# CederGroupHub/sparse-lm

Measured on AMD Instinct MI355X. Metric: fits/sec over 50-alpha Lasso path at n=100k p=5k, higher is better.
Workload: dtype f64

## Files before the change

sparse-lm_amd/csrc/engine_path.hip:

```cpp
#include "engine_internal.hpp"

static int ws_policy(const slm_host::Knobs& kn, const slm_dataset* ds, uint32_t flags) {
  if (ds->max_group > WS_KCAP / 2 || ds->n < 4) return 0;
  if (kn.ws == 0 || (flags & SLM_FLAG_NO_WORKING_SET)) return 0;
  const bool big = (double)ds->n * (double)ds->ld >= 67108864.0;
  return (big || (flags & SLM_FLAG_WORKING_SET) || kn.ws == 1) ? 2 : 1;
}

static bool small_ok(const slm_host::Knobs& kn, const slm_dataset* ds, uint32_t flags) {
  if (!(flags & SLM_FLAG_ON_CHIP)) return false;
  if (flags & (SLM_FLAG_NO_RESTART | SLM_FLAG_PROFILE | SLM_FLAG_FISTA_ONLY | SLM_FLAG_WORKING_SET | SLM_FLAG_NO_WORKING_SET))
    return false;
  if (!kn.on_chip) return false;
  return ds->p <= SM_PMAX && (double)ds->n * (double)ds->ld <= 131072.0 && !row_sharded(ds);
}
static bool split_possible(const slm_dataset* ds) {
  return ds->sk != nullptr && (ds->sk->rowdot != nullptr || !ds->XT_failed);
}
static int max_lanes_for(const slm_host::Knobs& kn, const slm_dataset* ds, uint32_t flags) {
  if (small_ok(kn, ds, flags)) return ds->lane_cap;
  if ((ws_policy(kn, ds, flags) == 2 || (double)ds->n * (double)ds->ld >= 67108864.0) && split_possible(ds)) {
    if (ws_policy(kn, ds, flags) == 2 && !row_sharded(ds) && ds->sk->rowdot != nullptr && !ds->XT_failed)
      return kMaxLanes;
    return SPLIT_LANES;
// ... 559 lines not shown
  ta.zprev = ds->zprev;
  ta.gprev = ds->gprev;
  ta.gscale = ds->gscale;
  ta.uscratch = ds->u;
  ta.a0 = ds->a0;
  ta.b0 = ds->b0;
  ta.d0 = ds->d0;
  ta.order = ds->order;
  ta.gid = ds->gid;
  ta.gstart = ds->gstart;
  ta.betas_out = ds->betas_out;
  ta.gn_out = any_gn ? ds->gn_out : nullptr;
  ta.infos = d_infos;

  return SLM_OK;
}

int PathCall::enqueue_result_copies() {
  int64_t at = 0;
  for (int l = 0; l < B;) {
    int l1 = l + 1;
    int64_t pts = lanes[l].n_points;
    const bool gn = lanes[l].group_norms_out != nullptr, inf = lanes[l].infos != nullptr;
    while (l1 < B && lanes[l1].betas_out == lanes[l].betas_out + (size_t)pts * p &&
           (lanes[l1].group_norms_out != nullptr) == gn && (lanes[l1].infos != nullptr) == inf &&
           (!gn || lanes[l1].group_norms_out == lanes[l].group_norms_out + (size_t)pts * G) &&
           (!inf || lanes[l1].infos == lanes[l].infos + pts)) {
      pts += lanes[l1].n_points;
      ++l1;
    }
    HIP_TRY(hipMemcpyAsync(lanes[l].betas_out, ds->betas_out + (size_t)at * p, sizeof(double) * (size_t)pts * p,
                           hipMemcpyDeviceToHost, s));
    if (gn)
      HIP_TRY(hipMemcpyAsync(lanes[l].group_norms_out, ds->gn_out + (size_t)at * G, sizeof(double) * (size_t)pts * G,
                             hipMemcpyDeviceToHost, s));
    if (inf && !infos_in_snap)
      HIP_TRY(hipMemcpyAsync(lanes[l].infos, ds->infos + at, sizeof(slm_point_info) * (size_t)pts,
                             hipMemcpyDeviceToHost, s));
    at += pts;
    l = l1;
  }
  return SLM_OK;
}

int PathCall::run_on_chip() {
  SmallArgs sm;
  memset(&sm, 0, sizeof(sm));
  sm.t = ta;
  sm.X = ds->X; sm.y = ds->y; sm.rw = ls.rw; sm.rw_stride = ls.rw_stride; sm.n = n;
  for (int l = 0; l < kMaxCells; ++l) sm.inv_n[l] = 1.0 / (ls.n_eff[l] > 0 ? ls.n_eff[l] : (double)ds->n_global);
  sm.max_iters = (int)std::min<int64_t>((int64_t)o.max_iter, 1500);
  sm.cold = (o.flags & SLM_FLAG_COLD_START) ? 1 : 0;
  const size_t fixed = sizeof(double) * ((size_t)p * p + 3 * (size_t)p);
  const size_t lds = (size_t)SM_LDS_BYTES;
  sm.stage_doubles = (int)((lds - fixed - 64) / sizeof(double));
  SLM_TRY(allow_big_lds((const void*)small_solve_kernel, eng->device));
  bool staged_out = (size_t)total_points * (size_t)p <= kSmallOutDoubles && !any_gn;
  if (staged_out && !ds->h_small_out &&
      hipHostMalloc((void**)&ds->h_small_out, sizeof(double) * kSmallOutDoubles, hipHostMallocDefault) != hipSuccess) {
    (void)hipGetLastError();
    ds->h_small_out = nullptr;
    staged_out = false;
  }
  if (staged_out) sm.t.betas_out = ds->h_small_out;
  hipLaunchKernelGGL(small_solve_kernel, dim3(B), dim3(SM_THREADS), lds, s, sm);
  SLM_TRY(check_launch());
  if (infos_in_snap) HIP_TRY(hipMemcpyAsync(&ds->hctl[0].c, ds->dctl, sizeof(DevCtl), hipMemcpyDeviceToHost, s));
  else HIP_TRY(hipMemcpyAsync(&ds->hctl[0].c, ds->dctl, offsetof(DevCtl, infos), hipMemcpyDeviceToHost, s));
  if (!staged_out) SLM_TRY(enqueue_result_copies());
  else if (!infos_in_snap) {
    int64_t at_i = 0;
    for (int l = 0; l < B; ++l) {
      if (lanes[l].infos)
        HIP_TRY(hipMemcpyAsync(lanes[l].infos, ds->infos + at_i, sizeof(slm_point_info) * (size_t)lanes[l].n_points, hipMemcpyDeviceToHost, s));
      at_i += lanes[l].n_points;
    }
  }
  HIP_TRY(hipStreamSynchronize(s));
  if (staged_out) {
    int64_t at_o = 0;
    for (int l = 0; l < B; ++l) {
      memcpy(lanes[l].betas_out, ds->h_small_out + (size_t)at_o * p, sizeof(double) * (size_t)lanes[l].n_points * p);
      at_o += lanes[l].n_points;
    }
  }
  const double t_small = t_mark();
  const DevCtl& snap = ds->hctl[0].c;
  bool nonfinite = false, unconverged = false;
  int64_t at = 0, sweeps = 0;
  std::vector<slm_point_info> far_infos;
  if (!infos_in_snap) {
    far_infos.resize((size_t)total_points);
    HIP_TRY(hipMemcpy(far_infos.data(), ds->infos, sizeof(slm_point_info) * (size_t)total_points, hipMemcpyDeviceToHost));
  }
  const slm_point_info* all = infos_in_snap ? snap.infos : far_infos.data();
  for (int l = 0; l < B; ++l) {
    nonfinite = nonfinite || snap.lane[l].nonfinite;
    sweeps += snap.lane[l].iter;
    for (int k = 0; k < lanes[l].n_points; ++k) unconverged = unconverged || all[at + k].status == SLM_ERR_NOT_CONVERGED;
    if (infos_in_snap && lanes[l].infos) memcpy(lanes[l].infos, snap.infos + at, sizeof(slm_point_info) * (size_t)lanes[l].n_points);
    at += lanes[l].n_points;
  }
  if (nonfinite) return fail(SLM_ERR_NON_FINITE, "non-finite iterate (diverged or non-finite data)");
  if (rules) {
    if (unconverged) return fail(SLM_ERR_UNSUPPORTED, "a re-weighted round was not settled on chip");
    for (int l = 0; l < B; ++l) {
      if (snap.lane[l].rounds < 1) return fail(SLM_ERR_UNSUPPORTED, "lane %d: the re-weighting rule covers no weight", l);
      rounds_out[l] = snap.lane[l].rounds;
    }
  }
  if (unconverged) {
    if (kn.trace == 2) fprintf(stderr, "[slm] on-chip solve gave a point up after %.3f ms (%lld products): the general path takes the call\n", t_small, (long long)sweeps);
    return solve_without_chip(kn, ds, lanes, B, o, stats, shared_path);
  }
  if (stats) {
    memset(stats, 0, sizeof(*stats));
    stats->grad_launches = 1;
    stats->ws_inner_iters = sweeps;
    stats->wall_ms = t_mark();
  }
  if (kn.trace == 2) {
      int sl = 0;
      double worst = -1.0;
      for (int l = 0; l < B; ++l) {
        const double t = snap.lane[l].hist[0] + snap.lane[l].hist[1] + snap.lane[l].hist[2] + snap.lane[l].hist[3] + snap.lane[l].hist[4];
        if (t > worst) { worst = t; sl = l; }
      }
      fprintf(stderr, "[slm] on-chip solve: row weights %.3f setup %.3f launched+synced %.3f end %.3f ms, %lld products; slowest lane (%d of %d, %d points, "
              "%d products, %d face solves) in the kernel: Gram %.3f, lambda_max %.3f, proximal steps %.3f, faces %.3f, records %.3f ms\n", tr_rw, tr[0],
              t_small, t_mark(), (long long)sweeps, sl, B, lanes[sl].n_points, snap.lane[sl].iter, (int)snap.lane[sl].n_hist, snap.lane[sl].hist[0],
              snap.lane[sl].hist[1], snap.lane[sl].hist[2], snap.lane[sl].hist[3], snap.lane[sl].hist[4]);
    }
  return SLM_OK;
}

int PathCall::ws_setup(bool late) {
  const int* set_of = ws_set_of;
  const int* set_lane = ws_set_lane;
  const int n_sets = ws_n_sets;
  const int ws_nblk_most = (int)std::max<int64_t>(1, std::min<int64_t>(eng->cus, n / 64));
  const bool share_blocks = ls.rw != nullptr && !sharded && n_sets > 1;
  const int ws_nblk = share_blocks ? std::max(1, std::min(ws_nblk_most, eng->cus - 2 * n_sets)) : ws_nblk_most;
  if (!ds->ws_idx) SLM_TRY(dalloc(&ds->ws_idx, WS_KCAP));
  if (!ds->ws_gs) SLM_TRY(dalloc(&ds->ws_gs, WS_KCAP));
  if (!ds->ws_gl) SLM_TRY(dalloc(&ds->ws_gl, WS_KCAP));
  if (!ds->ws_pos) SLM_TRY(dalloc(&ds->ws_pos, (size_t)ld));
  if (!ds->ws_score) SLM_TRY(dalloc(&ds->ws_score, (size_t)ld));
  if (!ds->ws_XW) SLM_TRY(dalloc(&ds->ws_XW, (size_t)n * WS_KCAP));
  if (!ds->ws_nt) SLM_TRY(dalloc(&ds->ws_nt, (size_t)kMaxLanes * NT_SCRATCH));
  if (ds->ws_sets < n_sets) {
    dfree(ds->ws_part); dfree(ds->ws_G); dfree(ds->ws_Gx);
    ds->ws_sets = 0;
    if (sharded) SLM_TRY(dalloc(&ds->ws_Gx, (size_t)n_sets * WS_KCAP * WS_KCAP + STOP_WORDS));
    SLM_TRY(dalloc(&ds->ws_part, (size_t)ws_nblk_most * n_sets * WS_KCAP * WS_KCAP));
    SLM_TRY(dalloc(&ds->ws_G, (size_t)n_sets * WS_KCAP * WS_KCAP));
    ds->ws_sets = n_sets;
  }
  SLM_TRY(ensure_xt(kn, ds));
  if (late) HIP_TRY(hipMemsetAsync(ds->ws_ctl, 0, sizeof(WsCtl), s));
  if (ws_carry && !late) hipLaunchKernelGGL(ws_ctl_carry_kernel, dim3(1), dim3(256), 0, s, ds->ws_ctl, kWsMaxBuilds);
  else if (late || !ws_begun) hipLaunchKernelGGL(ws_ctl_init_kernel, dim3(1), dim3(64), 0, s, ds->ws_ctl, kWsMaxBuilds);
  wa.ws = ds->ws_ctl;
  wa.idx = ds->ws_idx; wa.pos = ds->ws_pos; wa.gs = ds->ws_gs; wa.gl = ds->ws_gl;
  wa.score = ds->ws_score; wa.XW = ds->ws_XW; wa.part = ds->ws_part; wa.Gm = ds->ws_G;
  wa.nt = ds->ws_nt;
  if (sharded && !ds->ws_Gx) SLM_TRY(dalloc(&ds->ws_Gx, (size_t)ds->ws_sets * WS_KCAP * WS_KCAP + STOP_WORDS));
  wa.Gx = sharded ? ds->ws_Gx : nullptr;
  wa.X = ds->X; wa.XT = ds->XT; wa.n = n; wa.ld = ld;
  wa.rw = ls.rw; wa.rw_stride = ls.rw_stride;
  for (int l = 0; l < kMaxLanes; ++l) {
    wa.set_of[l] = l < B ? set_of[l] : 0;
    wa.set_lane[l] = l < n_sets ? set_lane[l] : 0;
    const int rep = wa.set_lane[l];
    wa.inv_n[l] = 1.0 / (ls.n_eff[rep] > 0 ? ls.n_eff[rep] : (double)ds->n_global);
  }
  wa.n_sets = n_sets;
  wa.nblk = ws_nblk;
  wa.owner = nullptr;
  if (ls.rw != nullptr && !sharded && kn.gram_owner && ws_nblk <= 512) {
    if (!ds->ws_owner) SLM_TRY(dalloc(&ds->ws_owner, (size_t)kMaxLanes * 512));
    hipLaunchKernelGGL(ws_block_owner_kernel, dim3((unsigned)ws_nblk), dim3(256), 0, s, ls.rw, ls.rw_stride, wa, ds->ws_owner);
    wa.owner = ds->ws_owner;
  }
  wa.theta = kn.ws_theta;
  wa.lookahead = slm_host::kWsLookahead;
  wa.append_max = kn.ws_append;
  wa.k_init = kn.ws_kinit > 0 ? kn.ws_kinit : (ds->singleton ? (shared_path ? 112 : 256) : 384);
  wa.bb_steps = kn.ws_bb;
  wa.one_solver = kn.ws_one_solver;
  wa.hard_call = kn.hard_callwide;
  wa.power_iters = slm_host::kWsPowerIters;
  wa.miss_factor = kn.ws_miss_factor;
  wa.miss_div = kn.ws_miss_div;
  wa.fill = kn.ws_fill > 0.0 ? kn.ws_fill : ((ds->singleton && shared_path) ? 0.75 : 0.5);
  return SLM_OK;
}

void PathCall::ws_release() {
  ds->ws_carry_valid = false;
  dfree(ds->ws_idx); dfree(ds->ws_pos); dfree(ds->ws_gs); dfree(ds->ws_gl);
  dfree(ds->ws_score); dfree(ds->ws_XW); dfree(ds->ws_part); dfree(ds->ws_G); dfree(ds->ws_Gx); dfree(ds->ws_nt);
  ds->ws_sets = 0;
  (void)hipGetLastError();
}

int PathCall::prepare_working_set() {
  {
    const int pol = ws_policy(kn, ds, o.flags);
    use_ws = pol == 2;
    ws_late = pol == 1 && !sharded;
  }
  if (sharded && !ds->stop_words) SLM_TRY(dalloc(&ds->stop_words, STOP_WORDS));
  if (use_ws) {
    const int rc = ws_setup(false);
    if (rc == SLM_ERR_OOM && !split && !sharded) {
      ws_release();
      use_ws = false;
    } else if (rc != SLM_OK) {
      return rc;
    }
  }
  done_flag = &ds->gctl->done;
  return SLM_OK;
}

int PathCall::enqueue_pass_gradient(hipEvent_t e0, hipEvent_t e1) {
  if (cov_on) return enqueue_gradient_cov(ds, B, cov_entry, done_flag, e0, e1, ds->ctl, use_ws ? &wa : nullptr);
  if (split) return enqueue_gradient_split(kn, ds, ls, ds->y, done_flag, ds->ctl, &wa, e0, e1, 0, (o.flags & SLM_FLAG_PROFILE_UNIT) != 0, light_skip);
  return enqueue_gradient(ds, ls, ds->y, done_flag, e0, e1, 0, light_skip);
}

void PathCall::enqueue_tail() {
  launch_tail(ta, s);
  if (shared_path && !interleave) hipLaunchKernelGGL(steal_kernel, dim3(1), dim3(256), 0, s, ta);
  if (shared_path && interleave && mg_handover) hipLaunchKernelGGL(tail_handover_kernel, dim3(1), dim3(64), 0, s, ta);
  else if (shared_path && interleave && use_ws && !ws_late && !sharded && planned_end > 0 && kn.lag_handover)
    hipLaunchKernelGGL(lag_handover_kernel, dim3(1), dim3(64), 0, s, ta, &ds->ws_ctl->builds, &ds->ws_ctl->stale, (int)(planned_end - enq - 1));
  if (sharded) {
    if (use_ws && wa.Gx) {
      hipLaunchKernelGGL(stop_pack_kernel, dim3(1), dim3(64), 0, s, ta.gdone, ds->ctl, B,
                         wa.Gx + (size_t)wa.n_sets * WS_KCAP * WS_KCAP);
    } else {
      hipLaunchKernelGGL(stop_pack_kernel, dim3(1), dim3(64), 0, s, ta.gdone, ds->ctl, B, ds->stop_words);
      if (ws_comm_rc == 0) ws_comm_rc = all_reduce_sum(eng, ds->stop_words, STOP_WORDS);
      hipLaunchKernelGGL(stop_apply_kernel, dim3(1), dim3(64), 0, s, ta.gdone, ds->stop_words);
    }
  }
}

void PathCall::enqueue_refinement() {
  if (use_ws) {
    {
      const int bs = ds->singleton ? 256 : 64;
      const int64_t items = ds->singleton ? p : 16 * (int64_t)G;
      hipLaunchKernelGGL(ws_score_kernel, dim3((unsigned)((items + bs - 1) / bs)), dim3(bs), 0, s, ta, wa);
      hipLaunchKernelGGL(ws_select_kernel, dim3(1), dim3(WS_THREADS), 0, s, ta, wa);
    }
    if (cov_on) {
      CovSets cs;
      for (int st = 0; st < kMaxLanes; ++st) cs.G[st] = st < wa.n_sets ? ds->cov[(size_t)cov_entry[wa.set_lane[st]]].G : nullptr;
      hipLaunchKernelGGL(ws_gram_cov_kernel, dim3(WS_TILES * WS_TILES, (unsigned)wa.n_sets), dim3(256), 0, s, wa, cs);
    } else {
    hipLaunchKernelGGL(ws_gather_kernel, dim3((unsigned)std::min<int64_t>((n + 31) / 32, 1024), WS_KCAP / 32), dim3(256), 0, s, wa);
    if (fix_start) {
      XtyArgs xa;
      xa.ws = wa.ws; xa.idx = wa.idx; xa.XW = wa.XW; xa.y = ds->y; xa.part = ds->partial; xa.g = ds->g; xa.gprev = ds->gprev; xa.z = ds->z;
      xa.ctl = ds->ctl; xa.done = done_flag; xa.n = n; xa.ld = ld; xa.inv_n = 1.0 / (double)ds->n_global; xa.n_lanes = B;
      xa.nblk = (int)std::max<int64_t>(1, std::min<int64_t>(2 * eng->cus, n / 64));
      hipLaunchKernelGGL(ws_xty_partial_kernel, dim3((unsigned)xa.nblk), dim3(512), 0, s, xa);
      hipLaunchKernelGGL(ws_xty_apply_kernel, dim3(WS_KCAP / 128), dim3(512), 0, s, xa);
    }
    hipLaunchKernelGGL(ws_gram_kernel, dim3((unsigned)wa.nblk, (unsigned)wa.n_sets, 1), dim3(WS_GRAM_THREADS), 0, s,
                       wa);
    if (wa.Gx)
      (void)hipMemsetAsync(wa.Gx, 0, sizeof(double) * (size_t)wa.n_sets * WS_KCAP * WS_KCAP, s);
    hipLaunchKernelGGL(ws_gram_reduce_kernel, dim3(WS_TILES * WS_TILES, (unsigned)wa.n_sets), dim3(256),
                       0, s, wa);
    }
    if (wa.Gx) {
      const size_t gram_words = (size_t)wa.n_sets * WS_KCAP * WS_KCAP;
      if (ws_comm_rc == 0) ws_comm_rc = all_reduce_sum(eng, wa.Gx, gram_words + STOP_WORDS);
      hipLaunchKernelGGL(ws_publish_kernel, dim3(WS_PUBLISH_BLOCKS, (unsigned)wa.n_sets), dim3(256), 0, s, wa);
      hipLaunchKernelGGL(stop_apply_kernel, dim3(1), dim3(64), 0, s, ta.gdone, wa.Gx + gram_words);
    }
    {
      if (wa.one_solver && wa.nt) {
      } else if (ds->singleton) hipLaunchKernelGGL((ws_solve_kernel<false, 0>), dim3(B), dim3(WS_THREADS), 0, s, ta, wa);
      else hipLaunchKernelGGL((ws_solve_kernel<true, 0>), dim3(B), dim3(WS_THREADS), 0, s, ta, wa);
      if (wa.nt) {
        if (ds->singleton) hipLaunchKernelGGL((ws_solve_kernel<false, 1>), dim3(B), dim3(WS_THREADS), 0, s, ta, wa);
        else hipLaunchKernelGGL((ws_solve_kernel<true, 1>), dim3(B), dim3(WS_THREADS), 0, s, ta, wa);
      }
    }
  }
}

void PathCall::plan_queue() {
  chunk = o.check_every;
  if (chunk <= 0) {
    const double est_us = std::max(12.0, (double)n * (double)ld * 8.0 / 5.0e6);
    chunk = est_us > 150.0 ? 2 : 4;
  }
  if (use_ws) chunk = std::min(chunk, 8);
  int max_points = 0;
  for (int l = 0; l < B; ++l) max_points = std::max(max_points, (int)lanes[l].n_points);
  if (shared_path) max_points = (int)total_points;
  max_total = (int64_t)max_points * o.max_iter;

  tr[2] = t_mark();
  if (use_ws && !ws_late && o.check_every <= 0) {
    int64_t most = 0;
    for (int l = 0; l < B; ++l) {
      int64_t mine = lanes[l].n_points;
      if (shared_path && interleave) mine = slm_host::interleaved_points(slm_host::LaneWalk{h[l].pt_lo, h[l].n_points, h[l].stride, h[l].tail_pt});
      most = std::max<int64_t>(most, mine);
    }
    expected = 1 + most;
    planned_end = expected;
  }
  {
    bool cold = true;
    for (int l = 0; l < B; ++l) cold = cold && lanes[l].beta0 == nullptr;
    if (cold && shared_path && use_ws && !ws_late && !sharded && !cov_on && split && !any_rw && !ds->rw &&
        !custom_scale && expected > 0 && o.max_iter >= 4 && !(o.flags & SLM_FLAG_FISTA_ONLY) && kn.sample_start) {
      const int64_t least = kn.sample_min_rows;
      if (n >= least) n_sample = n / kn.sample_div;
    }
  }
  mg_forced = kn.mg == 2;
  mg_cap = slm_host::model_gram_cap(ld, 3.0e9, kMgEntries);
  mg_ok = use_ws && split && (big_x || mg_forced) && !sharded && !cov_on && !(o.flags & SLM_FLAG_NO_MODEL_GRAM) &&
                     (size_t)ds->lane_cap >= (size_t)kMaxLanes && ws_n_sets <= mg_cap && mg_possible(kn, ds);
  if (mg_ok && mg_forced) expected = 0;
  if (mg_ok && !mg_forced && !ds->mg.empty()) {
    bool all = ws_n_sets > 0;
    for (int st = 0; st < ws_n_sets && all; ++st) {
      const int l = ws_set_lane[st];
      all = lanes[l].row_weight == nullptr;
      const double ne = ls.n_eff[l] > 0 ? ls.n_eff[l] : (double)ds->n_global;
      bool have = false;
      for (const auto& e : ds->mg) have = have || (e.own && e.n_eff == ne);
      all = all && have;
    }
    if (all) wa.keep_full = 1;
  }
  prof_off = n_sample > 0 ? 1 : 0;
  trace3 = kn.trace == 3;
  if (trace3 && kn.trace_poll && expected > 0) expected = n_sample > 0 ? 2 : 1;
}

int PathCall::mg_sets() {
  const double* wdev[SLM_MAX_LANES];
  double fp[2 * SLM_MAX_LANES] = {};
  int n_fp = 0, fp_at[SLM_MAX_LANES];
  for (int st = 0; st < ws_n_sets; ++st) {
    const int l = ws_set_lane[st];
    fp_at[st] = -1;
    if (lanes[l].row_weight != nullptr) {
      fp_at[st] = n_fp;
      wdev[n_fp++] = ls.rw + (int64_t)l * ls.rw_stride;
    }
  }
  if (n_fp > 0) SLM_TRY(cov_fingerprints(ds, wdev, n_fp, fp));
  int missing = 0;
  for (int pass = 0; pass < 2; ++pass) {
    if (pass == 1 && (int)ds->mg.size() + missing > mg_cap) mg_invalidate(ds);
    if (pass == 1) mg_built += missing;
    for (int st = 0; st < ws_n_sets; ++st) {
      const int l = ws_set_lane[st];
      const bool own = lanes[l].row_weight == nullptr;
      const double ne = ls.n_eff[l] > 0 ? ls.n_eff[l] : (double)ds->n_global;
      const double f1 = own ? 0.0 : fp[2 * fp_at[st]], f2 = own ? 0.0 : fp[2 * fp_at[st] + 1];
      if (pass == 0) {
        bool have = false;
        for (const auto& e : ds->mg) have = have || (e.n_eff == ne && (own ? e.own : (!e.own && e.fp1 == f1 && e.fp2 == f2)));
        missing += have ? 0 : 1;
      } else {
        SLM_TRY(mg_ensure(kn, ds, own ? nullptr : ls.rw + (int64_t)l * ls.rw_stride, ne, own, f1, f2, &mg_entry_of_set[st]));
      }
    }
  }
  return SLM_OK;
}

bool PathCall::mg_wanted(const DevCtl& c) const {
  if (mg_forced) return true;
  return c.ws.outgrown > 0 || c.ws.overflows > 0 || c.ws.disabled != 0;
}

int PathCall::mg_consider(const DevCtl& c) {
  if (!mg_ok || mg_on || !mg_wanted(c)) return SLM_OK;
  const auto t0 = std::chrono::steady_clock::now();
  const int rc = mg_sets();
  if (rc == SLM_OK) {
    mg_on = true;
    mg_handover = kn.handover;
    wa.keep_full = 1;
    if (mg_built > 0) mg_build_ms += std::chrono::duration<double, std::milli>(std::chrono::steady_clock::now() - t0).count();
  } else if (rc != SLM_ERR_OOM) {
    return rc;
  }
  return SLM_OK;
}

void PathCall::trace_pass(const DevCtl& now) const {
  if (!trace3) return;
  fprintf(stderr, "[slm] pass %lld at %.3f ms: K %d builds %d appends %d misses %d stale %d refined %d | mg on %d rounds %d inner %d most %d rej %d | light %d of %d (last: %d columns, why %d, D %.3g) | lanes (point.iter/flags):",
          (long long)enq, t_mark(), now.ws.Kreal, now.ws.builds, now.ws.appends, now.ws.misses, now.ws.stale, now.ws.refined, (int)mg_on,
          now.mg.rounds, now.mg.inner_iters, now.mg.most_iters, now.mg.rejected, now.lt.used, now.lt.attempts, now.lt.n_cols, now.lt.why, now.lt.D[0]);
  for (int l = 0; l < B; ++l)
    fprintf(stderr, " %d.%d%s%s%s", now.lane[l].point, now.lane[l].iter, now.lane[l].done ? "d" : "", now.lane[l].zsup ? "w" : "",
            l < SLM_MAX_LANES && now.mg.lane[l].active ? "m" : "");
  fprintf(stderr, "\n");
}

bool PathCall::light_eligible() {
  if (!kn.light_pass || !shared_path || !use_ws || ws_late || cov_on || sharded || mg_on) return false;
  if (any_rw || ds->rw || custom_scale || B > kMaxLanes || !(expected > 0 && enq >= expected)) return false;
  return ds->XT != nullptr && ds->XT_ready && ds->colnorm != nullptr && ds->colnorm_ready;
}

int PathCall::enqueue_light_attempt() {
  const int nblk = (int)std::max<int64_t>(std::max<int64_t>(1, std::min<int64_t>(eng->cus, n)), (n + 959) / 960);
  if (!ds->lt_dR) SLM_TRY(dalloc(&ds->lt_dR, (size_t)n * LT_LANES));
  if (!ds->lt_d2) SLM_TRY(dalloc(&ds->lt_d2, (size_t)nblk * (LT_LANES + kMaxLanes)));
  if (!ds->lt_part) SLM_TRY(dalloc(&ds->lt_part, (size_t)nblk * LT_CAP * LT_LANES));
  if (!ds->lt_cols) SLM_TRY(dalloc(&ds->lt_cols, (size_t)LT_CAP));
  if (!ds->lt_stamp) SLM_TRY(dalloc(&ds->lt_stamp, (size_t)ld));
  if (!light_begun) {
// ... 345 lines not shown
```

sparse-lm_amd/csrc/ws_kernels.hpp:

```cpp
#pragma once
#include <type_traits>
#include <hip/hip_runtime.h>
#include <stdint.h>

#include "tail_kernels.hpp"
#include "newton_kernels.hpp"

namespace slm {

constexpr int WS_KCAP = 512;
constexpr int WS_KLDS = 112;
constexpr int WS_TILES = WS_KCAP / 16;
constexpr int WS_THREADS = 1024;
constexpr int WS_INNER_MAX = 400;
constexpr int WS_BB_ITERS = 14;
constexpr double WS_BB_MAX_STEP = 20.0;
constexpr double WS_INNER_TOL = 0.05;
constexpr int WS_MAX_REPEATS = 6;
constexpr int WS_NEWTON_AFTER = 16;
constexpr int WS_NEWTON_MAX = 64;
constexpr int WS_AFTER_DIRECT = 40;
constexpr double WS_NEWTON_RQ = 0.05;
constexpr int WS_NEWTON_REFUSALS = 4;
constexpr double WS_NEWTON_ENTER = 0.3;
constexpr int WS_NEWTON_RESOLVE = 5;
static_assert(NT_MAXT * NT_B == WS_KCAP, "the direct solve covers a full working set");

struct WsCtl {
  int32_t request;
  int32_t building;
  int32_t valid;
  int32_t K;
  int32_t Kreal;
  int32_t k_new;
  int32_t builds;
  int32_t appends;
  int32_t max_builds;
  int32_t disabled;
  int32_t misses;
  int32_t refined;
  int32_t counter;
  int32_t stale;
  int32_t overflows;
  int32_t sweep_new;
  int32_t sweep_miss;
  int32_t staged;
  int32_t inner_iters;
  int32_t hard;
  int32_t hard_next;
  int32_t newton_steps;
  int32_t newton_fails;
  int32_t newton_nopd;
  int32_t newton_trial[4];
  int32_t newton_ref[4];
  int32_t newton_factors;
  int32_t newton_unknowns;
  unsigned long long nt_ticks[SLM_MAX_LANES][6];
  int32_t nt_factors[SLM_MAX_LANES];
  unsigned long long solve_ticks[5];
  int32_t want_full[SLM_MAX_LANES];
  int32_t iters_hist[32];
  unsigned long long lane_ticks[SLM_MAX_LANES];
  int32_t last_point[SLM_MAX_LANES];
  int32_t repeats[SLM_MAX_LANES];
  int32_t last_cols[SLM_MAX_LANES];
  double Lw[SLM_MAX_LANES];
  int32_t carried;
  int32_t outgrown;
  int32_t served[SLM_MAX_LANES];
  int32_t hard_lane[SLM_MAX_LANES];
};

struct WsArgs {
  WsCtl* ws;
  int32_t* idx;
  int32_t* pos;
  int32_t* gs;
  int32_t* gl;
  double* score;
  double* XW;
  double* part;
  double* Gm;
  double* nt;
  double* Gx;
  const double* X;
  const double* XT;
  int64_t n, ld;
  const double* rw;
  int64_t rw_stride;
  double inv_n[SLM_MAX_LANES];
  int32_t set_of[SLM_MAX_LANES];
  int32_t set_lane[SLM_MAX_LANES];
  int32_t n_sets;
  int32_t nblk;
  const int32_t* owner;
  double theta;
  int32_t lookahead;
  int32_t append_max;
  int32_t k_init;
  int32_t bb_steps;
  int32_t one_solver;
  int32_t miss_factor;
  int32_t miss_div;
  double fill;
  int32_t power_iters;
  int32_t hard_call;
  int32_t keep_full;
};

constexpr int WS_HEAD_WORDS = 24;
static_assert(offsetof(WsCtl, hard_next) / 4 < WS_HEAD_WORDS, "the words the pass kernels decide on");
#define WS_HEAD(hd, field) ((hd)[offsetof(WsCtl, field) / 4])
__device__ __forceinline__ void ws_head_load(const WsCtl* ws, const int* gdone, int32_t* hd) {
  const int tid = threadIdx.x;
  if (tid < WS_HEAD_WORDS) hd[tid] = reinterpret_cast<const int32_t*>(ws)[tid];
  else if (tid == WS_HEAD_WORDS) hd[tid] = gdone ? gdone[0] : 0;
}

static __global__ void ws_ctl_init_kernel(WsCtl* ws, int max_builds) {
  if (threadIdx.x == 0) {
    ws->request = 1;
    ws->max_builds = max_builds;
  }
  if (threadIdx.x < SLM_MAX_LANES) ws->last_point[threadIdx.x] = -1;
}

struct BeginArgs {
  const PathCtl* h_ctl;
  PathCtl* ctl;
  const slm_path_point* h_pts;
  slm_path_point* pts;
  int64_t n_pts;
  int32_t* head;
  int32_t head_words;
  const double* lambda;
  double margin;
  double factor[SLM_MAX_LANES];
  WsCtl* ws;
  int32_t max_builds;
  int32_t n_lanes;
};
static __global__ __launch_bounds__(256) void solve_begin_kernel(SetupArgs s, BeginArgs b) {
  solve_setup_body(s);
  const int64_t stride = (int64_t)gridDim.x * blockDim.x;
  {
    static_assert(sizeof(slm_path_point) == 4 * sizeof(double), "points travel as doubles");
    const double* src = reinterpret_cast<const double*>(b.h_pts);
    double* dst = reinterpret_cast<double*>(b.pts);
    for (int64_t e = (int64_t)blockIdx.x * blockDim.x + threadIdx.x; e < 4 * b.n_pts; e += stride) dst[e] = src[e];
  }
  if (blockIdx.x != 0) return;
  for (int e = threadIdx.x; e < b.head_words; e += 256) b.head[e] = 0;
  {
    static_assert(sizeof(PathCtl) % sizeof(int32_t) == 0, "control blocks travel as words");
    const int32_t* src = reinterpret_cast<const int32_t*>(b.h_ctl);
    int32_t* dst = reinterpret_cast<int32_t*>(b.ctl);
    const int words = b.n_lanes * (int)(sizeof(PathCtl) / sizeof(int32_t));
    for (int e = threadIdx.x; e < words; e += 256) dst[e] = src[e];
  }
  __syncthreads();
  if (b.lambda != nullptr && (int)threadIdx.x < b.n_lanes && threadIdx.x < SLM_MAX_LANES) {
    const int l = threadIdx.x;
    double L0 = b.lambda[0] * b.margin;
    if (L0 <= 0.0) L0 = 1.0;
    const double L = L0 * b.factor[l];
// ... 505 lines not shown
#pragma unroll
        for (int c = 0; c < C; ++c) acc[c] = __builtin_fma(lane + 64 * c < K ? xv[r][c] : 0.0, yv[r], acc[c]);
      }
    }
  };
  switch ((K + 63) >> 6) {
    case 1: rows4(std::integral_constant<int, 1>{}); break;
    case 2: rows4(std::integral_constant<int, 2>{}); break;
    case 3: rows4(std::integral_constant<int, 3>{}); break;
    case 4: rows4(std::integral_constant<int, 4>{}); break;
    case 5: rows4(std::integral_constant<int, 5>{}); break;
    case 6: rows4(std::integral_constant<int, 6>{}); break;
    case 7: rows4(std::integral_constant<int, 7>{}); break;
    default: rows4(std::integral_constant<int, 8>{}); break;
  }
  static_assert(WS_KCAP / 64 == 8, "eight chunks of 64 positions");
#pragma unroll
  for (int c = 0; c < WS_KCAP / 64; ++c) red[wave][lane + 64 * c] = acc[c];
  if (lane == 0) red_yy[wave] = yy;
  __syncthreads();
  double* out = a.part + (int64_t)blockIdx.x * (WS_KCAP + 1);
  const int k = threadIdx.x;
  if (k < K) {
    double sum = 0.0;
#pragma unroll
    for (int w = 0; w < 8; ++w) sum += red[w][k];
    out[k] = sum;
  }
  if (k == WS_KCAP - 1) {
    double sum = 0.0;
#pragma unroll
    for (int w = 0; w < 8; ++w) sum += red_yy[w];
    out[WS_KCAP] = sum;
  }
}
static __global__ __launch_bounds__(512) void ws_xty_apply_kernel(XtyArgs a) {
  if (*a.done) return;
  __shared__ double red[4][128];
  __shared__ double ry[512];
  const int K = a.ws->K;
  const int kl = threadIdx.x & 127, q = threadIdx.x >> 7;
  const int k = (int)blockIdx.x * 128 + kl;
  if ((int)blockIdx.x * 128 >= K) return;
  double s[8] = {0, 0, 0, 0, 0, 0, 0, 0};
  if (k < K) {
    int b = q;
    for (; b + 28 < a.nblk; b += 32) {
#pragma unroll
      for (int u = 0; u < 8; ++u) s[u] += a.part[(int64_t)(b + 4 * u) * (WS_KCAP + 1) + k];
    }
    for (; b < a.nblk; b += 4) s[0] += a.part[(int64_t)b * (WS_KCAP + 1) + k];
  }
  red[q][kl] = ((s[0] + s[1]) + (s[2] + s[3])) + ((s[4] + s[5]) + (s[6] + s[7]));
  if (blockIdx.x == 0) ry[threadIdx.x] = (int)threadIdx.x < a.nblk ? a.part[(int64_t)threadIdx.x * (WS_KCAP + 1) + WS_KCAP] : 0.0;
  __syncthreads();
  if (q == 0 && k < K) {
    const int j = a.idx[k];
    if (j >= 0) {
      const double c = -((red[0][kl] + red[1][kl]) + (red[2][kl] + red[3][kl])) * a.inv_n;
      for (int l = 0; l < a.n_lanes; ++l) {
        a.g[(int64_t)l * (a.ld + 16) + j] = c;
        a.gprev[(int64_t)l * a.ld + j] = c;
        a.z[(int64_t)l * a.ld + j] = 0.0;
      }
    }
  }
  if (blockIdx.x == 0) {
    for (int off = 256; off >= 1; off >>= 1) {
      if ((int)threadIdx.x < off) ry[threadIdx.x] += ry[threadIdx.x + off];
      __syncthreads();
    }
    if (threadIdx.x < (unsigned)a.n_lanes) {
      const int l = threadIdx.x;
      const double loss0 = 0.5 * ry[0] * a.inv_n;
      a.g[(int64_t)l * (a.ld + 16) + a.ld] = loss0;
      a.ctl[l].hist[0] = loss0;
      a.ctl[l].loss_base = loss0;
    }
  }
}

static __global__ __launch_bounds__(256) void ws_block_owner_kernel(const double* rw, int64_t rw_stride, WsArgs w, int32_t* owner) {
  __shared__ int cls[SLM_MAX_LANES];
  __shared__ int red[2][4];
  const int tid = threadIdx.x;
  const int64_t b = blockIdx.x;
  const int64_t base = w.n / w.nblk, rem = w.n % w.nblk;
  const int64_t r0 = b * base + (b < rem ? b : rem);
  const int64_t nrows = base + (b < rem ? 1 : 0);
  for (int st = 0; st < w.n_sets; ++st) {
    const double* v = rw + (int64_t)w.set_lane[st] * rw_stride + r0;
    int zeros = 1, ones = 1;
    for (int64_t i = tid; i < nrows; i += 256) {
      const double x = v[i];
      zeros &= (x == 0.0);
      ones &= (x == 1.0);
    }
    zeros = __all(zeros);
    ones = __all(ones);
    if ((tid & 63) == 0) {
      red[0][tid >> 6] = zeros;
      red[1][tid >> 6] = ones;
    }
    __syncthreads();
    if (tid == 0) {
      const int z = red[0][0] & red[0][1] & red[0][2] & red[0][3], o = red[1][0] & red[1][1] & red[1][2] & red[1][3];
      cls[st] = z ? 0 : (o ? 1 : 2);
    }
    __syncthreads();
  }
  if (tid == 0) {
    int first_ones = -1;
    for (int st = 0; st < w.n_sets; ++st) {
      int o = st;
      if (cls[st] == 0) o = -1;
      else if (cls[st] == 1) {
        if (first_ones < 0) first_ones = st;
        o = first_ones;
      }
      owner[(int64_t)st * w.nblk + b] = o;
    }
  }
}

typedef double ws_d4 __attribute__((ext_vector_type(4)));
constexpr int WS_GRAM_THREADS = 512;
constexpr int WS_GRAM_ZCHUNKS = 4;

static __global__ __launch_bounds__(WS_GRAM_THREADS) void ws_gram_kernel(WsArgs w) {
  if (!w.ws->building) return;
  __shared__ ws_d4 comb[2][16][64];
  const int K = w.ws->K;
  const int tile_lo = w.ws->k_new >> 4;
  const int tid = threadIdx.x, lane = tid & 63;
  const int wave = __builtin_amdgcn_readfirstlane(tid >> 6);
  const int tiles = K >> 4;
  const bool row_split = (tile_lo > 0 || tiles <= 8) && tiles - tile_lo <= 4 * WS_GRAM_ZCHUNKS;
  const int set = blockIdx.y;
  const int64_t b = blockIdx.x;
  if (w.owner != nullptr && w.owner[(int64_t)set * w.nblk + b] != set) return;
  const int64_t base = w.n / w.nblk, rem = w.n % w.nblk;
  const int64_t r0 = b * base + (b < rem ? b : rem);
  const int64_t nrows = base + (b < rem ? 1 : 0);
  const double* rw = w.rw ? w.rw + (int64_t)w.set_lane[set] * w.rw_stride : nullptr;
  const int part = row_split ? (wave >> 1) : 0;
  const int64_t steps = (nrows + 3) >> 2;
  const int64_t s_begin = row_split ? 4 * (steps * part / 4) : 0;
  const int64_t s_end = row_split ? min(nrows, 4 * (steps * (part + 1) / 4)) : nrows;

  for (int slice = 0; slice < 4 * WS_GRAM_ZCHUNKS; ++slice) {
  const int zhi = slice >> 2;
  if (8 * (slice & 3) >= tiles) continue;
  if (row_split ? (tile_lo + 4 * zhi >= tiles) : (zhi >= 2)) continue;
  const int wj = 2 * (slice & 3) + (wave & 1);
  const int ntj = min(4, max(0, tiles - 4 * wj));
  const int ibase = row_split ? tile_lo + 4 * zhi : 4 * (4 * zhi + (wave >> 1));
  const int ti_lo = row_split ? 0 : max(0, tile_lo - ibase);
  const int nti = min(4, max(0, tiles - ibase));
  const bool active = ti_lo < nti && ntj > 0;
  if (!row_split && !active) continue;
  ws_d4 acc[4][4];
#pragma unroll
  for (int ti = 0; ti < 4; ++ti)
#pragma unroll
    for (int tj = 0; tj < 4; ++tj) acc[ti][tj] = ws_d4{0.0, 0.0, 0.0, 0.0};

  const int kk = lane >> 4, c = lane & 15;
  if (active) {
    const int ta_max = WS_TILES - 1;
    const double* rwp = rw ? rw : w.XW;
    const bool has_rw = rw != nullptr;
    auto load = [&](int64_t s, double(&av)[4], double(&bv)[4], double& wgt) {
      const int64_t i = s + kk;
      const bool ok = i < s_end;
      const int64_t row = r0 + (ok ? i : 0);
      const double wv = rwp[has_rw ? row : 0];
      const double* xr = w.XW + row * WS_KCAP + c;
#pragma unroll
      for (int t = 0; t < 4; ++t) {
        av[t] = xr[16 * min(ibase + t, ta_max)];
        bv[t] = xr[16 * min(4 * wj + t, ta_max)];
      }
      wgt = ok ? (has_rw ? wv : 1.0) : 0.0;
    };
    auto mma = [&](const double(&av)[4], const double(&bv)[4], double wgt) {
#pragma unroll
      for (int ti = 0; ti < 4; ++ti) {
        if (ti >= ti_lo && ti < nti) {
          const double a = av[ti] * wgt;
#pragma unroll
          for (int tj = 0; tj < 4; ++tj)
            if (tj < ntj) acc[ti][tj] = __builtin_amdgcn_mfma_f64_16x16x4f64(a, bv[tj], acc[ti][tj], 0, 0, 0);
        }
      }
    };
    double a0[4], b0[4], a1[4], b1[4], a2[4], b2[4], a3[4], b3[4], w0, w1, w2, w3;
    load(s_begin, a0, b0, w0);
    load(s_begin + 4, a1, b1, w1);
    load(s_begin + 8, a2, b2, w2);
    for (int64_t s = s_begin; s < s_end; s += 16) {
      load(s + 12, a3, b3, w3);
      mma(a0, b0, w0);
      load(s + 16, a0, b0, w0);
      mma(a1, b1, w1);
      load(s + 20, a1, b1, w1);
      mma(a2, b2, w2);
      load(s + 24, a2, b2, w2);
      mma(a3, b3, w3);
    }
  }
  if (row_split) {
    for (int round = 0; round < 4; ++round) {
      if (part == round && active) {
#pragma unroll
        for (int ti = 0; ti < 4; ++ti)
#pragma unroll
          for (int tj = 0; tj < 4; ++tj) {
            if (ti < nti && tj < ntj) {
              if (round > 0) acc[ti][tj] += comb[wave & 1][ti * 4 + tj][lane];
              if (round < 3) comb[wave & 1][ti * 4 + tj][lane] = acc[ti][tj];
            }
          }
      }
      __syncthreads();
    }
  }
  if (!row_split || (part == 3 && active)) {
#pragma unroll
  for (int ti = 0; ti < 4; ++ti) {
    if (ti < ti_lo || ti >= nti) continue;
#pragma unroll
    for (int tj = 0; tj < 4; ++tj) {
      if (tj >= ntj) continue;
      const int64_t tile = (int64_t)(ibase + ti) * WS_TILES + (4 * wj + tj);
      double* out = w.part + (((int64_t)set * (WS_TILES * WS_TILES) + tile) * w.nblk + b) * 256;
#pragma unroll
      for (int r = 0; r < 4; ++r) out[(kk + 4 * r) * 16 + c] = acc[ti][tj][r];
    }
  }
  }
  if (row_split) __syncthreads();
  }
}

static __global__ __launch_bounds__(256) void ws_gram_reduce_kernel(WsArgs w) {
  WsCtl* ws = w.ws;
  if (!ws->building) return;
  const int K = ws->K;
  const int row_lo = (ws->k_new >> 4) << 4;
  const int set = blockIdx.y;
  const int tile = blockIdx.x, I = tile / WS_TILES, J = tile % WS_TILES;
  const int tiles = K >> 4, I_lo = row_lo >> 4;
  if (I < I_lo || I >= tiles || J >= tiles) return;
  const int i = 16 * I + (threadIdx.x >> 4), j = 16 * J + (threadIdx.x & 15);
  {
    const double* src = w.part + (((int64_t)set * (WS_TILES * WS_TILES) + tile) * w.nblk) * 256 + threadIdx.x;
    double s4[4] = {0.0, 0.0, 0.0, 0.0};
    int b = 0;
    if (w.owner != nullptr) {
      __shared__ int64_t off_s[512];
      static_assert(sizeof(off_s) >= 8 * 512, "nblk <= 512");
      for (int bb = threadIdx.x; bb < w.nblk; bb += 256) {
        const int o = w.owner[(int64_t)set * w.nblk + bb];
        off_s[bb] = o < 0 ? -1 : (int64_t)(o - set) * (WS_TILES * WS_TILES) * w.nblk * 256;
      }
      __syncthreads();
      for (; b + 32 <= w.nblk; b += 32) {
        double v[32];
#pragma unroll
        for (int u = 0; u < 32; ++u) {
          const int64_t o = off_s[b + u];
          v[u] = o == -1 ? 0.0 : src[(int64_t)(b + u) * 256 + o];
        }
#pragma unroll
        for (int u = 0; u < 32; ++u) s4[u & 3] += v[u];
      }
      for (; b < w.nblk; ++b) {
        const int64_t o = off_s[b];
        s4[b & 3] += o == -1 ? 0.0 : src[(int64_t)b * 256 + o];
      }
    }
    for (; b + 32 <= w.nblk; b += 32) {
      double v[32];
#pragma unroll
      for (int u = 0; u < 32; ++u) v[u] = src[(int64_t)(b + u) * 256];
#pragma unroll
      for (int u = 0; u < 32; ++u) s4[u & 3] += v[u];
    }
    for (; b < w.nblk; ++b) s4[b & 3] += src[(int64_t)b * 256];
    double s = ((s4[0] + s4[1]) + (s4[2] + s4[3])) * w.inv_n[set];
    double* Gs = (w.Gx ? w.Gx : w.Gm) + (int64_t)set * (WS_KCAP * WS_KCAP);
    Gs[i * WS_KCAP + j] = s;
    if (j < row_lo) Gs[j * WS_KCAP + i] = s;
  }
  __threadfence();
  __syncthreads();
  if (threadIdx.x == 0) {
    const int total = (tiles - I_lo) * tiles * (int)gridDim.y;
    if (atomicAdd(&ws->counter, 1) + 1 == total) {
      ws->counter = 0;
      if (w.Gx) {
        ws->staged = 1;
      } else {
        ws->request = 0;
        ws->valid = 1;
        __threadfence();
        ws->building = 0;
      }
    }
  }
}

constexpr int WS_PUBLISH_BLOCKS = 64;
static __global__ __launch_bounds__(256) void ws_publish_kernel(WsArgs w) {
  WsCtl* ws = w.ws;
  if (!ws->building || !ws->staged) return;
  const int K = ws->K;
  const int row_lo = (ws->k_new >> 4) << 4;
  const int set = blockIdx.y;
  for (int i = blockIdx.x; i < K; i += gridDim.x)
    for (int j = threadIdx.x; j < K; j += 256)
      if (i >= row_lo || j >= row_lo) {
        const int64_t at = (int64_t)set * (WS_KCAP * WS_KCAP) + (int64_t)i * WS_KCAP + j;
        w.Gm[at] = w.Gx[at];
      }
  __threadfence();
  __syncthreads();
  if (threadIdx.x == 0) {
    const int total = gridDim.x * gridDim.y;
    if (atomicAdd(&ws->counter, 1) + 1 == total) {
      ws->counter = 0;
      ws->staged = 0;
      ws->request = 0;
      ws->valid = 1;
      __threadfence();
      ws->building = 0;
    }
  }
}

template <int NV>
__device__ __forceinline__ void ws_sum(double (&v)[NV], double (*lds)[TAIL_WAVES], int nwc) {
  const int lane = threadIdx.x & 63;
  const int wave = __builtin_amdgcn_readfirstlane(threadIdx.x >> 6);
  if (wave < nwc) {
#pragma unroll
    for (int k = 0; k < NV; ++k) v[k] = wave_sum_lane63(v[k]);
  }
  __syncthreads();
  if (wave < nwc && lane == 63) {
#pragma unroll
    for (int k = 0; k < NV; ++k) lds[k][wave] = v[k];
  }
  __syncthreads();
  if (nwc == 4) {
#pragma unroll
    for (int k = 0; k < NV; ++k) v[k] = group_sum_all<4>(lds[k][lane & 3]);
  } else {
#pragma unroll
    for (int k = 0; k < NV; ++k) v[k] = group_sum_all<8>(lds[k][lane & 7]);
  }
}

struct WsSolveLds {
  double delta[WS_KCAP];
  double uim[WS_KCAP];
  double part[WS_THREADS];
  double Gl[WS_KLDS * WS_KLDS];
  NtShared nts;
  double nv[WS_KCAP];
  double xsl[WS_KCAP];
  double rgl[WS_KCAP];
  double pbl[WS_KCAP];
  double scale2;
  int nz[WS_KCAP];
  int act[WS_KCAP];
  int rank_of[WS_KCAP];
  int nnz, m;
};

template <bool GROUPED, bool DIRECT>
__device__ __forceinline__ bool ws_refine_lane(TailArgs a, const WsArgs& w, double (*red)[TAIL_WAVES], WsSolveLds& sh) {
  double (&delta)[WS_KCAP] = sh.delta;
  double (&uim)[WS_KCAP] = sh.uim;
  int (&nz)[WS_KCAP] = sh.nz;
  int& nnz_s = sh.nnz;
  double (&part)[WS_THREADS] = sh.part;
  double (&Gl)[WS_KLDS * WS_KLDS] = sh.Gl;
  NtShared& nts = sh.nts;
  double (&nv)[WS_KCAP] = sh.nv;
  int (&act)[WS_KCAP] = sh.act;
  int (&rank_of)[WS_KCAP] = sh.rank_of;
  int& m_s = sh.m;
  double (&xsl)[WS_KCAP] = sh.xsl;
  double (&rgl)[WS_KCAP] = sh.rgl;
  double (&pbl)[WS_KCAP] = sh.pbl;
  double& scale2_s = sh.scale2;
  const int lane_id = blockIdx.x;
  PathCtl* ctl = a.ctl + lane_id;
  WsCtl* ws = w.ws;
  if (!ws->valid || ws->building || ws->disabled) return true;
  const int tid = threadIdx.x;
  const int p = a.p;
  const int K = __builtin_amdgcn_readfirstlane(ws->K);
  const int set = w.set_of[lane_id];
  const double* Gm = w.Gm + (int64_t)set * (WS_KCAP * WS_KCAP);
  {
    const int64_t off = (int64_t)lane_id * a.ld;
    a.beta += off; a.z += off; a.zprev += off; a.gprev += off;
    a.a0 += off; a.b0 += off; a.d0 += off;
    a.pts += ctl->pt_off;
  }
  if (ws->stale) {
    double out[1] = {0.0};
    for (int j = tid; j < p; j += WS_THREADS)
      if (w.pos[j] < 0 && a.z[j] != a.zprev[j]) out[0] += 1.0;
    block_sum<1>(out, red);
    if (out[0] != 0.0) return true;
  }
  const int point_now = ctl->point + ctl->pt_off;
  const int reps = (ws->last_point[lane_id] == point_now && ws->last_cols[lane_id] == ws->Kreal) ? ws->repeats[lane_id] : 0;
  if (reps >= WS_MAX_REPEATS) return true;
  const int hard_now = w.hard_call ? ws->hard : ws->hard_lane[lane_id];
  if (!DIRECT && w.nt != nullptr && hard_now != 0) {
    if (tid == 0) ws->want_full[lane_id] = 1;
    return false;
  }

  unsigned long long tk_s = wall_clock64();
  auto mark = [&](int slot) {
    if (tid == 0 && lane_id == 0) {
      const unsigned long long now = wall_clock64();
      ws->solve_ticks[slot] += now - tk_s;
      tk_s = now;
    }
  };
  const slm_path_point pt = a.pts[ctl->point];
  const int mode = ctl->mode;
  const double tol = ctl->tol;
  const bool group_pen = (pt.sb != 0.0) || (pt.sd != 0.0);
  const bool g_lds = K <= WS_KLDS;
  if (g_lds) {
    for (int e = tid; e < K * K; e += WS_THREADS) {
      const int r = e / K, c = e - r * K;
      Gl[e] = Gm[r * WS_KCAP + c];
    }
  }

  const int tsh = K <= 256 ? 2 : 1;
  const int TPC = 1 << tsh;
  const int KP = WS_THREADS >> tsh;
// ... 891 lines not shown
```

Measured before the change: 17170.

## Compute only lower-triangular Gram tiles and mirror them in the reduce

The working-set Gram kernel now skips MFMA work and partial-sum stores for tiles above the diagonal. The partial buffer and the reduce grid shrink to the triangular tile count, and the reduce writes each element to both symmetric positions. This roughly halves the Gram compute and the partial-buffer traffic. The cost is more indexing logic, including a linear search for the triangular index, plus some wave-assignment swizzling in the row-split path.

```diff
diff --git a/sparse-lm_amd/csrc/engine_path.hip b/sparse-lm_amd/csrc/engine_path.hip
--- a/sparse-lm_amd/csrc/engine_path.hip
+++ b/sparse-lm_amd/csrc/engine_path.hip
@@ -735,7 +735,7 @@
     dfree(ds->ws_part); dfree(ds->ws_G); dfree(ds->ws_Gx);
     ds->ws_sets = 0;
     if (sharded) SLM_TRY(dalloc(&ds->ws_Gx, (size_t)n_sets * WS_KCAP * WS_KCAP + STOP_WORDS));
-    SLM_TRY(dalloc(&ds->ws_part, (size_t)ws_nblk_most * n_sets * WS_KCAP * WS_KCAP));
+    SLM_TRY(dalloc(&ds->ws_part, (size_t)ws_nblk_most * n_sets * WS_TRI_TILES * 256));
     SLM_TRY(dalloc(&ds->ws_G, (size_t)n_sets * WS_KCAP * WS_KCAP));
     ds->ws_sets = n_sets;
   }
@@ -857,7 +857,7 @@
                        wa);
     if (wa.Gx)
       (void)hipMemsetAsync(wa.Gx, 0, sizeof(double) * (size_t)wa.n_sets * WS_KCAP * WS_KCAP, s);
-    hipLaunchKernelGGL(ws_gram_reduce_kernel, dim3(WS_TILES * WS_TILES, (unsigned)wa.n_sets), dim3(256),
+    hipLaunchKernelGGL(ws_gram_reduce_kernel, dim3(WS_TRI_TILES, (unsigned)wa.n_sets), dim3(256),
                        0, s, wa);
     }
     if (wa.Gx) {
diff --git a/sparse-lm_amd/csrc/ws_kernels.hpp b/sparse-lm_amd/csrc/ws_kernels.hpp
--- a/sparse-lm_amd/csrc/ws_kernels.hpp
+++ b/sparse-lm_amd/csrc/ws_kernels.hpp
@@ -11,6 +11,7 @@
 constexpr int WS_KCAP = 512;
 constexpr int WS_KLDS = 112;
 constexpr int WS_TILES = WS_KCAP / 16;
+constexpr int WS_TRI_TILES = WS_TILES * (WS_TILES + 1) / 2;
 constexpr int WS_THREADS = 1024;
 constexpr int WS_INNER_MAX = 400;
 constexpr int WS_BB_ITERS = 14;
@@ -822,12 +823,14 @@
   const int zhi = slice >> 2;
   if (8 * (slice & 3) >= tiles) continue;
   if (row_split ? (tile_lo + 4 * zhi >= tiles) : (zhi >= 2)) continue;
-  const int wj = 2 * (slice & 3) + (wave & 1);
+  const int wj = 2 * (slice & 3) + ((wave & 1) ^ (row_split ? (zhi & 1) : 0));
   const int ntj = min(4, max(0, tiles - 4 * wj));
   const int ibase = row_split ? tile_lo + 4 * zhi : 4 * (4 * zhi + (wave >> 1));
+  if (row_split && 8 * (slice & 3) > min(tiles - 1, ibase + 3)) continue;
   const int ti_lo = row_split ? 0 : max(0, tile_lo - ibase);
   const int nti = min(4, max(0, tiles - ibase));
-  const bool active = ti_lo < nti && ntj > 0;
+  auto lower = [&](int ti, int tj) { return 4 * wj + tj <= ibase + ti; };
+  const bool active = ti_lo < nti && ntj > 0 && lower(nti - 1, 0);
   if (!row_split && !active) continue;
   ws_d4 acc[4][4];
 #pragma unroll
@@ -860,7 +863,7 @@
           const double a = av[ti] * wgt;
 #pragma unroll
           for (int tj = 0; tj < 4; ++tj)
-            if (tj < ntj) acc[ti][tj] = __builtin_amdgcn_mfma_f64_16x16x4f64(a, bv[tj], acc[ti][tj], 0, 0, 0);
+            if (tj < ntj && lower(ti, tj)) acc[ti][tj] = __builtin_amdgcn_mfma_f64_16x16x4f64(a, bv[tj], acc[ti][tj], 0, 0, 0);
         }
       }
     };
@@ -886,7 +889,7 @@
         for (int ti = 0; ti < 4; ++ti)
 #pragma unroll
           for (int tj = 0; tj < 4; ++tj) {
-            if (ti < nti && tj < ntj) {
+            if (ti < nti && tj < ntj && lower(ti, tj)) {
               if (round > 0) acc[ti][tj] += comb[wave & 1][ti * 4 + tj][lane];
               if (round < 3) comb[wave & 1][ti * 4 + tj][lane] = acc[ti][tj];
             }
@@ -901,9 +904,10 @@
     if (ti < ti_lo || ti >= nti) continue;
 #pragma unroll
     for (int tj = 0; tj < 4; ++tj) {
-      if (tj >= ntj) continue;
-      const int64_t tile = (int64_t)(ibase + ti) * WS_TILES + (4 * wj + tj);
-      double* out = w.part + (((int64_t)set * (WS_TILES * WS_TILES) + tile) * w.nblk + b) * 256;
+      if (tj >= ntj || !lower(ti, tj)) continue;
+      const int I = ibase + ti;
+      const int64_t tile = (int64_t)I * (I + 1) / 2 + (4 * wj + tj);
+      double* out = w.part + (((int64_t)set * WS_TRI_TILES + tile) * w.nblk + b) * 256;
 #pragma unroll
       for (int r = 0; r < 4; ++r) out[(kk + 4 * r) * 16 + c] = acc[ti][tj][r];
     }
@@ -919,12 +923,15 @@
   const int K = ws->K;
   const int row_lo = (ws->k_new >> 4) << 4;
   const int set = blockIdx.y;
-  const int tile = blockIdx.x, I = tile / WS_TILES, J = tile % WS_TILES;
+  const int tile = blockIdx.x;
+  int I = 0;
+  while ((I + 1) * (I + 2) / 2 <= tile) ++I;
+  const int J = tile - I * (I + 1) / 2;
   const int tiles = K >> 4, I_lo = row_lo >> 4;
-  if (I < I_lo || I >= tiles || J >= tiles) return;
+  if (I < I_lo || I >= tiles) return;
   const int i = 16 * I + (threadIdx.x >> 4), j = 16 * J + (threadIdx.x & 15);
   {
-    const double* src = w.part + (((int64_t)set * (WS_TILES * WS_TILES) + tile) * w.nblk) * 256 + threadIdx.x;
+    const double* src = w.part + (((int64_t)set * WS_TRI_TILES + tile) * w.nblk) * 256 + threadIdx.x;
     double s4[4] = {0.0, 0.0, 0.0, 0.0};
     int b = 0;
     if (w.owner != nullptr) {
@@ -932,7 +939,7 @@
       static_assert(sizeof(off_s) >= 8 * 512, "nblk <= 512");
       for (int bb = threadIdx.x; bb < w.nblk; bb += 256) {
         const int o = w.owner[(int64_t)set * w.nblk + bb];
-        off_s[bb] = o < 0 ? -1 : (int64_t)(o - set) * (WS_TILES * WS_TILES) * w.nblk * 256;
+        off_s[bb] = o < 0 ? -1 : (int64_t)(o - set) * WS_TRI_TILES * w.nblk * 256;
       }
       __syncthreads();
       for (; b + 32 <= w.nblk; b += 32) {
@@ -960,13 +967,15 @@
     for (; b < w.nblk; ++b) s4[b & 3] += src[(int64_t)b * 256];
     double s = ((s4[0] + s4[1]) + (s4[2] + s4[3])) * w.inv_n[set];
     double* Gs = (w.Gx ? w.Gx : w.Gm) + (int64_t)set * (WS_KCAP * WS_KCAP);
-    Gs[i * WS_KCAP + j] = s;
-    if (j < row_lo) Gs[j * WS_KCAP + i] = s;
+    if (j <= i) {
+      Gs[i * WS_KCAP + j] = s;
+      Gs[j * WS_KCAP + i] = s;
+    }
   }
   __threadfence();
   __syncthreads();
   if (threadIdx.x == 0) {
-    const int total = (tiles - I_lo) * tiles * (int)gridDim.y;
+    const int total = (tiles * (tiles + 1) - I_lo * (I_lo + 1)) / 2 * (int)gridDim.y;
     if (atomicAdd(&ws->counter, 1) + 1 == total) {
       ws->counter = 0;
       if (w.Gx) {
```

Result: no change. 17240 (median of 6 runs) (+0.4%).
